# AlexGr5/StereoVision

Hardware: AMD Instinct MI355X
Metric: disparity frames/sec + HBM GB/s, 1920x1080 D=128 win=9, 1/2/4/8 GPU (higher is better)
Workload: dtype u8

## Files before the change

stereovision_amd/csrc/sv_capi_dev.cpp:

```cpp
#include "sv_ctx.h"

extern "C" {

int sv_gray_dev(sv_ctx* c, const uint8_t* d_bgr, int H, int W, int pitch, uint8_t* d_gray, void* stream) {
    SV_ENTER(c);
    if (check_image(d_bgr, H, W) || !d_gray) return fail(SV_EINVAL, "bad gray arguments");
    hipStream_t s = pick(c, stream);
    SV_LAUNCH(c, SV_K_GRAY, s, sv::launch_gray(d_bgr, H, W, pitch, d_gray, s));
    return 0;
}

int sv_disparity_dev(sv_ctx* c, const uint8_t* d_left, const uint8_t* d_right, int H, int W, int pitch,
                     int min_disp, int num_disp, int win, int cost, int row0, int row1, int16_t* d_disp16,
                     int out_pitch, void* stream) {
    SV_ENTER(c);
    if (check_image(d_left, H, W) || check_image(d_right, H, W) || !d_disp16)
        return fail(SV_EINVAL, "bad disparity arguments");
    if (pitch < W || out_pitch < W) return fail(SV_EINVAL, "pitch smaller than width");
    hipStream_t s = pick(c, stream);
    SV_SCRATCH(c, s);
    return enqueue_disparity(c, d_left, d_right, H, W, pitch, min_disp, num_disp, win, cost, row0, row1,
                             d_disp16, out_pitch, s);
}

int sv_median_rows_dev(sv_ctx* c, const int16_t* d_disp16, int H, int W, int row0, int row1, int min_disp,
                       int num_disp, int cost, const sv_map_out* out, void* stream) {
    SV_ENTER(c);
    if (check_image(d_disp16, H, W)) return fail(SV_EINVAL, "bad median arguments");
    if ((long long)H * W >= (1LL << 30)) return fail(SV_EINVAL, "frame too large for the median kernel");
    if (row0 < 0) row0 = 0;
    if (row1 > H) row1 = H;
    hipStream_t s = pick(c, stream);
    SV_SCRATCH(c, s);
    sv::PostParams pp;
    float* disp = nullptr;
    int rc = map_out_post(c, out, min_disp, num_disp, cost, false, s, &pp, &disp);
    if (rc) return rc;
    SV_LAUNCH(c, SV_K_MEDIAN, s, sv::launch_median_i16(d_disp16, H, W, row0, row1, disp, pp, s));
    return 0;
}

int sv_post_m16_dev(sv_ctx* c, const int16_t* d_med16, int64_t n, int mode, float min_depth, float max_depth,
                    float depth_range, float min_disp_global, int min_disp, int num_disp, float* d_disparity,
                    float* d_out_a, uint8_t* d_out_u8, float* d_out_b, void* stream) {
    SV_ENTER(c);
    if (n < 0 || (n > 0 && !d_med16)) return fail(SV_EINVAL, "bad median map");
    if (mode != SV_POST_NONE && mode != SV_POST_DEPTH && mode != SV_POST_SCALED) return fail(SV_EINVAL, "bad mode");
    if (mode == SV_POST_NONE && !d_disparity) return fail(SV_EINVAL, "no outputs");
    if (mode == SV_POST_DEPTH && (!d_out_a || !d_out_u8)) return fail(SV_EINVAL, "depth post outputs missing");
    if (mode == SV_POST_SCALED && (!d_out_a || !d_out_u8 || !d_out_b || num_disp <= 0))
        return fail(SV_EINVAL, "scaled post outputs missing");
    if (n == 0) return 0;
    hipStream_t s = pick(c, stream);
    SV_SCRATCH(c, s);
    sv::PostParams pp = make_post(mode, min_depth, max_depth, depth_range, min_disp_global, min_disp, num_disp,
                                  d_out_a, d_out_u8, d_out_b);
    int rc = attach_lut(c, pp, s);
    if (rc) return rc;
    SV_LAUNCH(c, SV_K_POST, s, sv::launch_post_m16(d_med16, (long long)n, d_disparity, pp, s));
    return 0;
}

int sv_disparity_batch_dev(sv_ctx* c, const uint8_t* d_left, const uint8_t* d_right, int n_frames, int H,
                           int W, int pitch, int64_t frame_stride, int min_disp, int num_disp, int win,
                           int cost, int16_t* d_disp16, int out_pitch, int64_t out_frame_stride,
                           void* stream) {
    SV_ENTER(c);
    if (check_image(d_left, H, W) || check_image(d_right, H, W) || !d_disp16 || n_frames < 0)
        return fail(SV_EINVAL, "bad disparity arguments");
    if (pitch < W || out_pitch < W) return fail(SV_EINVAL, "pitch smaller than width");
    if (n_frames > 1 && (frame_stride < (int64_t)pitch * H || out_frame_stride < (int64_t)out_pitch * H))
        return fail(SV_EINVAL, "frame stride smaller than a frame");
    if (n_frames == 0) return 0;
    hipStream_t s = pick(c, stream);
    SV_SCRATCH(c, s);
    return enqueue_disparity(c, d_left, d_right, H, W, pitch, min_disp, num_disp, win, cost, 0, H, d_disp16,
                             out_pitch, s, n_frames, frame_stride, out_frame_stride);
}

int sv_depth_map_batch_dev(sv_ctx* c, const uint8_t* d_left, const uint8_t* d_right, int n_frames, int H, int W,
                           int pitch, int64_t frame_stride, int min_disp, int num_disp, int win, int cost, int stages,
                           int16_t* d_disp16, const sv_map_out* out, void* stream) {
    SV_ENTER(c);
    if (stages != SV_STAGE_ALL && stages != SV_STAGE_MATCH && stages != SV_STAGE_MEDIAN)
        return fail(SV_EINVAL, "stages must be SV_STAGE_MATCH, SV_STAGE_MEDIAN or SV_STAGE_ALL");
    const bool match = stages & SV_STAGE_MATCH, median = stages & SV_STAGE_MEDIAN;
    if (n_frames < 0 || H <= 0 || W <= 0) return fail(SV_EINVAL, "bad depth-map arguments");
    if (match && (check_image(d_left, H, W) || check_image(d_right, H, W)))
        return fail(SV_EINVAL, "bad depth-map arguments");
    if (!d_disp16 && stages != SV_STAGE_ALL)
        return fail(SV_EINVAL, "the stages run apart exchange the int16 maps through d_disp16");
    if (median && !out) return fail(SV_EINVAL, "null outputs");
    if (median && out->harris && check_image(d_left, H, W)) return fail(SV_EINVAL, "Harris needs the left frames");
    if (pitch < W) return fail(SV_EINVAL, "pitch smaller than width");
    if (n_frames > 1 && frame_stride < (int64_t)pitch * H) return fail(SV_EINVAL, "frame stride smaller than a frame");
    if ((long long)H * W >= (1LL << 30)) return fail(SV_EINVAL, "frame too large for the median kernel");
    if (n_frames == 0) return 0;
    hipStream_t s = pick(c, stream);
    SV_SCRATCH(c, s);
    const long long fs = (long long)H * W;
    int16_t* d16 = d_disp16;
    if (!d16) {
        SV_HIP(c->d16.ensure((size_t)n_frames * fs * sizeof(int16_t)));
        d16 = c->d16.as<int16_t>();
    }
    if (match) {
        const int rc = enqueue_disparity(c, d_left, d_right, H, W, pitch, min_disp, num_disp, win, cost, 0, H, d16, W,
                                         s, n_frames, frame_stride, fs, !d_disp16);
        if (rc) return rc;
    }
    if (!median) return 0;
    sv::PostParams pp;
    float* disp = nullptr;
    int rc = map_out_post(c, out, min_disp, num_disp, cost, true, s, &pp, &disp);
    if (rc) return rc;
    pp.lut_unchecked = match && cost != SV_COST_SGBM && pp.lut_shift == 4 && pp.lut_m0 == (min_disp - 1) * 16 &&
                       pp.lut_n == num_disp + 1;
    const long long fin = n_frames > 1 ? frame_stride : 0;
    if (out->harris && (W < 8 || H < 8)) {
        SV_LAUNCH(c, SV_K_MEDIAN, s, sv::launch_median_i16(d16, H, W, 0, H, disp, pp, s, n_frames, fs, fs));
        SV_LAUNCH(c, SV_K_HARRIS, s, sv::launch_harris(d_left, H, W, pitch, out->harris, s, n_frames, fin, fs));
        return 0;
    }
    sv::HarrisParams hp{d_left, pitch, fin, out->harris, fs, 0, 0};
    SV_LAUNCH(c, SV_K_MEDIAN, s,
              sv::launch_median_i16(d16, H, W, 0, H, disp, pp, s, n_frames, fs, fs, out->harris ? &hp : nullptr));
    return 0;
}

int sv_harris_dev(sv_ctx* c, const uint8_t* d_gray, int H, int W, int pitch, float* d_out, void* stream) {
    SV_ENTER(c);
    if (check_image(d_gray, H, W) || !d_out) return fail(SV_EINVAL, "bad harris arguments");
    hipStream_t s = pick(c, stream);
    SV_LAUNCH(c, SV_K_HARRIS, s, sv::launch_harris(d_gray, H, W, pitch, d_out, s));
    return 0;
}

int sv_harris_batch_dev(sv_ctx* c, const uint8_t* d_gray, int n_frames, int H, int W, int pitch,
                        int64_t frame_stride, float* d_out, void* stream) {
    SV_ENTER(c);
    if (check_image(d_gray, H, W) || !d_out || n_frames < 0) return fail(SV_EINVAL, "bad harris arguments");
    if (pitch < W) return fail(SV_EINVAL, "pitch smaller than width");
    if (n_frames > 1 && frame_stride < (int64_t)pitch * H) return fail(SV_EINVAL, "frame stride smaller than a frame");
    if (n_frames == 0) return 0;
    hipStream_t s = pick(c, stream);
    SV_LAUNCH(c, SV_K_HARRIS, s,
              sv::launch_harris(d_gray, H, W, pitch, d_out, s, n_frames, (long long)frame_stride,
                                (long long)H * W));
    return 0;
}

int sv_hog_hist_dev(sv_ctx* c, const uint8_t* d_gray, int H, int W, int pitch, int win, int row0, int row1,
                    uint16_t* d_out, void* stream) {
    SV_ENTER(c);
    if (check_image(d_gray, H, W) || !d_out) return fail(SV_EINVAL, "bad hog arguments");
    if (win < 1 || win > 15 || (win & 1) == 0) return fail(SV_EINVAL, "win must be odd in [1, 15]");
    hipStream_t s = pick(c, stream);
    SV_LAUNCH(c, SV_K_HOG, s, sv::launch_hog_hist(d_gray, H, W, pitch, win, row0, row1, d_out, s));
    return 0;
}

int sv_gray(sv_ctx* c, const uint8_t* bgr, int H, int W, int stride, uint8_t* gray) {
    SV_ENTER(c);
    SV_SCRATCH(c, c->stream);
    if (check_image(bgr, H, W) || !gray) return fail(SV_EINVAL, "bad gray arguments");
    const size_t row = (size_t)W * 3, n = row * H;
    if (stride < (int)row) return fail(SV_EINVAL, "stride smaller than a row");
    SV_HIP(c->hin.ensure(n));
    for (int y = 0; y < H; ++y) std::memcpy(c->hin.as<uint8_t>() + y * row, bgr + (size_t)y * stride, row);
    SV_HIP(c->img[0].ensure(n));
    SV_HIP(c->gray[0].ensure((size_t)H * W));
    SV_HIP(hipMemcpyAsync(c->img[0].p, c->hin.p, n, hipMemcpyHostToDevice, c->stream));
    SV_LAUNCH(c, SV_K_GRAY, c->stream,
              sv::launch_gray(c->img[0].as<uint8_t>(), H, W, (int)row, c->gray[0].as<uint8_t>(), c->stream));
    Out o[] = {{gray, c->gray[0].p, (size_t)H * W}};
    return collect(c, o, 1);
}

int sv_disparity(sv_ctx* c, const uint8_t* left, const uint8_t* right, int H, int W, int channels, int stride,
                 int min_disp, int num_disp, int win, int cost, int16_t* disp16, float* harris) {
    SV_ENTER(c);
    SV_SCRATCH(c, c->stream);
    if (!disp16) return fail(SV_EINVAL, "null disparity output");
    sv::MatchPlan plan;
    int rc = check_match(H, W, min_disp, num_disp, win, cost, &plan);
    if (rc) return rc;
    rc = stage_pair(c, left, right, H, W, channels, stride);
    if (rc) return rc;
    SV_HIP(c->d16.ensure((size_t)H * W * sizeof(int16_t)));
    rc = enqueue_disparity(c, c->gray[0].as<uint8_t>(), c->gray[1].as<uint8_t>(), H, W, W, min_disp, num_disp,
                           win, cost, 0, H, c->d16.as<int16_t>(), W, c->stream);
    if (rc) return rc;
    if (harris) {
        SV_HIP(c->harris.ensure((size_t)H * W * sizeof(float)));
        SV_LAUNCH(c, SV_K_HARRIS, c->stream,
                  sv::launch_harris(c->gray[0].as<uint8_t>(), H, W, W, c->harris.as<float>(), c->stream));
    }
    Out o[] = {{disp16, c->d16.p, (size_t)H * W * sizeof(int16_t)},
               {harris, c->harris.p, (size_t)H * W * sizeof(float)}};
    return collect(c, o, 2);
}

int sv_disparity_rows(sv_ctx* c, const uint8_t* left, const uint8_t* right, int H, int W, int channels,
                      int stride, int min_disp, int num_disp, int win, int cost, int row0, int row1,
                      int16_t* disp16) {
    SV_ENTER(c);
    SV_SCRATCH(c, c->stream);
    if (!disp16) return fail(SV_EINVAL, "null disparity output");
    if (row0 < 0) row0 = 0;
    if (row1 > H) row1 = H;
    if (row1 <= row0) return 0;
    sv::MatchPlan plan;
    int rc = check_match(H, W, min_disp, num_disp, win, cost, &plan);
    if (rc) return rc;
    rc = stage_pair(c, left, right, H, W, channels, stride);
    if (rc) return rc;
    SV_HIP(c->d16.ensure((size_t)H * W * sizeof(int16_t)));
    rc = enqueue_disparity(c, c->gray[0].as<uint8_t>(), c->gray[1].as<uint8_t>(), H, W, W, min_disp, num_disp,
                           win, cost, row0, row1, c->d16.as<int16_t>(), W, c->stream);
    if (rc) return rc;
    const size_t off = (size_t)row0 * W;
    Out o[] = {{disp16 + off, c->d16.as<int16_t>() + off, (size_t)(row1 - row0) * W * sizeof(int16_t)}};
    return collect(c, o, 1);
}


int sv_median5_f32(sv_ctx* c, const float* in, int H, int W, float* out) {
    SV_ENTER(c);
    SV_SCRATCH(c, c->stream);
    if (check_image(in, H, W) || !out) return fail(SV_EINVAL, "bad median arguments");
    const size_t n = (size_t)H * W * sizeof(float);
    SV_HIP(c->hin.ensure(n));
    SV_HIP(c->fin.ensure(n));
    SV_HIP(c->fa.ensure(n));
    std::memcpy(c->hin.p, in, n);
    SV_HIP(hipMemcpyAsync(c->fin.p, c->hin.p, n, hipMemcpyHostToDevice, c->stream));
    SV_LAUNCH(c, SV_K_MEDIAN, c->stream, sv::launch_median_f32(c->fin.as<float>(), H, W, c->fa.as<float>(), c->stream));
    Out o[] = {{out, c->fa.p, n}};
    return collect(c, o, 1);
}

static int post_common(sv_ctx* c, const float* disparity, int n, const sv::PostParams& tmpl, float* a,
                       uint8_t* u8, float* b) {
    if (!disparity || n <= 0) return fail(SV_EINVAL, "bad post arguments");
    const size_t nb = (size_t)n * sizeof(float);
    SV_HIP(c->hin.ensure(nb));
    SV_HIP(c->fin.ensure(nb));
    SV_HIP(c->fa.ensure(nb));
    SV_HIP(c->fb.ensure(nb));
    SV_HIP(c->u8.ensure((size_t)n));
    std::memcpy(c->hin.p, disparity, nb);
    SV_HIP(hipMemcpyAsync(c->fin.p, c->hin.p, nb, hipMemcpyHostToDevice, c->stream));
    sv::PostParams pp = tmpl;
    pp.out_a = c->fa.as<float>();
    pp.out_u8 = c->u8.as<uint8_t>();
    pp.out_b = c->fb.as<float>();
    SV_LAUNCH(c, SV_K_POST, c->stream, sv::launch_post(c->fin.as<float>(), n, pp, c->stream));
    Out o[] = {{a, c->fa.p, nb}, {u8, c->u8.p, (size_t)n}, {b, c->fb.p, nb}};
    return collect(c, o, 3);
}

int sv_depth_post(sv_ctx* c, const float* disparity, int n, float min_depth, float max_depth, float depth_range,
                  float min_disp_global, float* depth_final, uint8_t* depth_normalized) {
    SV_ENTER(c);
    SV_SCRATCH(c, c->stream);
    if (!depth_final || !depth_normalized) return fail(SV_EINVAL, "null outputs");
    sv::PostParams pp = make_post(SV_POST_DEPTH, min_depth, max_depth, depth_range, min_disp_global, 0, 0,
                                  nullptr, nullptr, nullptr);
    return post_common(c, disparity, n, pp, depth_final, depth_normalized, nullptr);
}

int sv_scaled_post(sv_ctx* c, const float* disparity, int n, int min_disp, int num_disp,
                   float* disparity_normalized, uint8_t* normalized_u8, float* confidence) {
    SV_ENTER(c);
    SV_SCRATCH(c, c->stream);
    if (!disparity_normalized || !normalized_u8 || !confidence || num_disp <= 0)
        return fail(SV_EINVAL, "bad scaled post arguments");
    sv::PostParams pp = make_post(SV_POST_SCALED, 0.f, 0.f, 0.f, 0.f, min_disp, num_disp, nullptr, nullptr,
                                  nullptr);
    return post_common(c, disparity, n, pp, disparity_normalized, normalized_u8, confidence);
}

}

namespace {

std::mutex g_reg_mu;
std::map<uintptr_t, size_t> g_reg;

bool host_registered(const void* p, size_t bytes) {
    if (!p) return false;
    const uintptr_t a = reinterpret_cast<uintptr_t>(p);
    std::lock_guard<std::mutex> lk(g_reg_mu);
    auto it = g_reg.upper_bound(a);
    if (it == g_reg.begin()) return false;
    --it;
    return a >= it->first && a + bytes <= it->first + it->second;
}

int stage_rows(sv_ctx* c, const uint8_t* src, int y0, int y1, size_t row, int stride, uint8_t* stage, uint8_t* dev,
               int nsub) {
    if ((size_t)stride == row) {
        SV_HIP(hipMemcpyAsync(dev + (size_t)y0 * row, src + (size_t)y0 * row, (size_t)(y1 - y0) * row,
                              hipMemcpyHostToDevice, c->stream));
        return 0;
    }
    sv::HostPool& pool = sv::HostPool::get();
    for (int k = 0; k < nsub; ++k) {
        const int a0 = y0 + (int)((long long)(y1 - y0) * k / nsub), a1 = y0 + (int)((long long)(y1 - y0) * (k + 1) / nsub);
        if (a1 <= a0) continue;
        const int parts = pool.threads();
        pool.parallel_for(parts, [&](int p) {
            const int a = a0 + (int)((long long)(a1 - a0) * p / parts), b = a0 + (int)((long long)(a1 - a0) * (p + 1) / parts);
            if (b <= a) return;
            if ((size_t)stride == row)
                std::memcpy(stage + (size_t)a * row, src + (size_t)a * row, (size_t)(b - a) * row);
            else
                for (int y = a; y < b; ++y) std::memcpy(stage + (size_t)y * row, src + (size_t)y * stride, row);
        });
        SV_HIP(hipMemcpyAsync(dev + (size_t)a0 * row, stage + (size_t)a0 * row, (size_t)(a1 - a0) * row,
                              hipMemcpyHostToDevice, c->stream));
    }
    return 0;
}

int host_lut(sv_ctx* c, const sv::PostParams& pp) {
    if (c->hl_valid && c->hl_key == c->lut_key) return 0;
    const size_t n = (size_t)pp.lut_n;
    try {
        c->hl_a.resize(n);
        c->hl_b.resize(n);
        c->hl_u8.resize(n);
    } catch (...) {
        return fail(SV_ENOMEM, "host table allocation failed");
    }
    SV_HIP(hipMemcpyAsync(c->hl_a.data(), pp.lut_a, n * sizeof(float), hipMemcpyDeviceToHost, c->stream));
    SV_HIP(hipMemcpyAsync(c->hl_b.data(), pp.lut_b, n * sizeof(float), hipMemcpyDeviceToHost, c->stream));
    SV_HIP(hipMemcpyAsync(c->hl_u8.data(), pp.lut_u8, n, hipMemcpyDeviceToHost, c->stream));
    SV_HIP(hipStreamSynchronize(c->stream));
    c->hl_key = c->lut_key;
    c->hl_valid = true;
    return 0;
}

struct FrameOut {
    float* a;
    float* disp;
    uint8_t* u8;
    float* b;
    uint8_t* bgr;
};

template <bool U8, bool SCALED, bool BGR>
int expand_rows(const int16_t* med, size_t a, size_t b, int m0, int nl, const HostEnt* ent, const float* lb,
                const FrameOut& o) {
    for (size_t i = a; i < b; ++i) o.disp[i] = (float)med[i] * 0.0625f;
    int nbad = 0;
    for (size_t i = a; i < b; ++i) {
        const uint32_t li = (uint32_t)(med[i] - m0);
        if (__builtin_expect(li >= (uint32_t)nl, 0)) {
            ++nbad;
            continue;
        }
        const HostEnt e = ent[li];
        o.a[i] = e.a;
        if (U8) o.u8[i] = (uint8_t)e.ubgr;
        if (SCALED) o.b[i] = lb[li];
        if (BGR) {
            const uint32_t v = e.ubgr >> 8;
            uint8_t* d = o.bgr + 3 * i;
            if (i + 1 < b) std::memcpy(d, &v, 4);
            else std::memcpy(d, &v, 3);
        }
    }
    return nbad;
}

struct HostProf {
    std::atomic<bool> on{std::getenv("SV_HOST_PROFILE") != nullptr};
    bool print = std::getenv("SV_HOST_PROFILE") != nullptr;
    std::mutex mu;
    double t[6] = {0, 0, 0, 0, 0, 0};
    double acc[6] = {0, 0, 0, 0, 0, 0};
    long n = 0, nacc = 0;
    void add(const double* d) {
        std::lock_guard<std::mutex> lk(mu);
        for (int i = 0; i < 6; ++i) {
            t[i] += d[i];
            acc[i] += d[i];
        }
        ++nacc;
        if (print && ++n % 200 == 0) {
            std::fprintf(stderr, "[sv host] per call (ms): prepare %.3f  stage+issue %.3f  wait-first %.3f  expand %.3f  "
                         "wait-rest %.3f  total %.3f\n", t[0] / n, t[1] / n, t[2] / n, t[3] / n, t[4] / n, t[5] / n);
            for (double& v : t) v = 0;
            n = 0;
        }
    }
};
HostProf& host_prof() {
    static HostProf* p = new HostProf();
    return *p;
}
int env_int(const char* name, int dflt, int lo, int hi) {
    const char* e = std::getenv(name);
    if (!e) return dflt;
    const int v = std::atoi(e);
    return v < lo ? lo : v > hi ? hi : v;
}
double now_ms() {
    return std::chrono::duration<double, std::milli>(std::chrono::steady_clock::now().time_since_epoch()).count();
}

int host_frame_path(sv_ctx* c, const uint8_t* left, const uint8_t* right, int H, int W, int channels, int stride,
                    int min_disp, int num_disp, int win, int cost, sv::PostParams pp, const uint8_t* table,
                    FrameOut o) {
    const bool prof = host_prof().on;
    double tm[6] = {0, 0, 0, 0, 0, 0}, t0 = prof ? now_ms() : 0, tp = t0;
    sv::MatchPlan plan;
    int rc = check_match(H, W, min_disp, num_disp, win, cost, &plan);
// ... 861 lines not shown
```

stereovision_amd/csrc/sv_internal.h:

```cpp
#pragma once
#include <hip/hip_runtime.h>
#include <stdint.h>

#include <cstdlib>
#include <string>

struct sv_comm;

namespace sv {

__device__ __forceinline__ void sad_u32_acc(uint32_t& a, uint32_t b, uint32_t c) {
    asm("v_sad_u32 %0, %0, %1, %2" : "+v"(a) : "v"(b), "v"(c));
}

__device__ __forceinline__ int clampi(int v, int lo, int hi) { return min(max(v, lo), hi); }

__device__ __forceinline__ int bgr_to_gray(int b, int g, int r) {
    return (b * 1868 + g * 9617 + r * 4899 + (1 << 13)) >> 14;
}

inline bool env_flag(const char* name, bool default_on) {
    const char* e = std::getenv(name);
    return default_on ? !(e && e[0] == '0') : (e && e[0] == '1');
}
inline int env_int(const char* name, int lo, int hi) {
    const char* e = std::getenv(name);
    const int v = e ? std::atoi(e) : 0;
    return v >= lo && v <= hi ? v : 0;
}

int set_error(int code, const std::string& msg);

int comm_group_start();
int comm_group_end();
int comm_send(sv_comm* c, const void* buf, size_t bytes, int peer, hipStream_t s);
int comm_recv(sv_comm* c, void* buf, size_t bytes, int peer, hipStream_t s);
int comm_rank(const sv_comm* c);
int comm_size(const sv_comm* c);
int comm_device(const sv_comm* c);

enum Cost { COST_SAD = 0, COST_SSD = 1, COST_HOG = 2, COST_SGBM = 3 };

struct MatchPlan {
    int dpl;
    int lpg;
    int ndw;
    int dbits;
    int mfma_only = 0;
};

struct MatchParams {
    const uint8_t* L;
    const uint8_t* R;
    const uint16_t* HL;
    const uint16_t* HR;
    int H, W, pitch;
    int minD, D, r;
    int win;
    int X0, X1;
    int row0, row1;
    int lpg, lpg_log2, dbits;
    int16_t* out;
    int opitch;
    int nf;
    long long fs_in, fs_out, fs_hist;
    uint32_t pad_key;
    int segm;
    alignas(16) int xcd_map;
    uint32_t* keys;
    long long keys_stride;
    int margins_done;
};

int plan_match(int num_disp, int win, int cost, MatchPlan* plan);
uint64_t max_cost(int win, int cost);
size_t match_lds_bytes(const MatchPlan& p, int r, int cost);
int launch_match(const MatchParams& a, const MatchPlan& p, int cost, hipStream_t s);
bool ring_split(int cost, int win, int num_disp);
bool ring_ssd(int cost, int win, int num_disp);
bool ssd_mfma(int cost, int win, int num_disp);
bool ssd_mfma_fits(const MatchParams& a, int cost);
int launch_ssd_mfma(const MatchParams& a, hipStream_t s);
long long ring_split_elems(int nf, long long fs_out, int row1, int opitch);
int launch_fill_i16(int16_t* out, int opitch, int H, int W, int16_t v, hipStream_t s);

int launch_gray(const uint8_t* bgr, int H, int W, int pitch, uint8_t* gray, hipStream_t s);
int launch_harris(const uint8_t* g, int H, int W, int pitch, float* out, hipStream_t s, int nf = 1,
                  long long fs_in = 0, long long fs_out = 0);
int launch_hog_hist(const uint8_t* g, int H, int W, int pitch, int win, int row0, int row1,
                    uint16_t* hist, hipStream_t s);
int launch_hog_hist_pairs(const uint8_t* g0, const uint8_t* g1, int H, int W, int pitch, int win, int row0,
                          int row1, uint16_t* h0, uint16_t* h1, int nf, long long fs_in, long long fs_hist,
                          hipStream_t s);

struct UndistortParams {
    double ir[9];
    double fx, fy, u0, v0;
    double k[12];
    int H, W;
};
int launch_undistort_map(const UndistortParams& p, short2* map1, uint16_t* map2, hipStream_t s);
int launch_remap(const uint8_t* src, int sH, int sW, int channels, int spitch, long long sfs,
                 const short2* map1, const uint16_t* map2, int H, int W, bool gray_out, uint8_t* dst,
                 int dpitch, long long dfs, int nf, hipStream_t s);

int launch_resize_linear(const void* src, int sH, int sW, int cn, int spitch, long long sfs, void* dst,
                         int dH, int dW, int dpitch, long long dfs, int nf, bool f32, hipStream_t s);

struct FrameStatsArgs {
    const uint8_t* img0;
    const uint8_t* img1;
    int H, W, pitch, cn;
    int bh, bw;
    uint32_t* block_sum;
    uint32_t* block_sq;
    uint32_t* hist;
    uint32_t* hist_copies;
    int per;
    long long fs;
};
constexpr int kHistCopies = 8;
int launch_frame_stats(const FrameStatsArgs& a, int nimg, hipStream_t s);

enum SelectMask { SEL_ALL = 0, SEL_POSITIVE = 1, SEL_MASK_GT = 2 };
constexpr int kMaxRanks = 4;
constexpr int kSelBatch = 16;
struct SelectArgs {
    const float* x;
    const float* mask;
    float thr;
    int mask_mode;
    size_t n;
    int shift, bits;
    int nranks;
    int narr;
    size_t xstride, mstride;
    uint32_t prefix[kSelBatch][kMaxRanks];
    uint32_t* ghist;
    unsigned long long* counts;
    uint32_t* hist_out;
    unsigned long long* counts_out;
};
constexpr int kCountSlots = 32;
int launch_select_hist(const SelectArgs& a, hipStream_t s);

enum AffineMode { AFF_F32 = 0, AFF_F64 = 1, AFF_FILL = 2 };
struct AffineArgs {
    const float* x;
    float* out;
    size_t n;
    int mode;
    float fa, fb, fc, fd;
    double ds, doff;
};
int launch_affine_f32(const AffineArgs& a, hipStream_t s);

struct GaussArgs {
    const float* src;
    float* dst;
    int H, W, r;
    float c[16];
};
enum FuseBase { FUSE_BASE_STEREO = 0, FUSE_BASE_MIDAS = 1, FUSE_BASE_FLOW = 2 };
struct FuseBlendArgs {
    const float* stereo;
    const float* conf;
    const float* midas;
    const float* flow;
    float* fused;
    uint32_t* stats;
    int H, W, base;
    int midas_fill, flow_fill;
    int r;
    float sw, mfw, thr, hthr, k1, k2;
    float c[16];
};
constexpr int kBilateralMaxR = 7;
constexpr int kBilateralMaxTaps = 148;
constexpr int kBilateralLut = 4096 + 2;
struct BilateralArgs {
    const float* src;
    const float* lut;
    float* dst_f32;
    uint8_t* dst_u8;
    uint8_t* dst_bgr;
    const uint32_t* cmap;
    uint32_t* stats;
    int H, W, r, ntaps;
    float scale;
    float sw[kBilateralMaxTaps];
    short off[kBilateralMaxTaps];
};
int bilateral_taps(int r, int* dy, int* dx);
int launch_gauss_f32(const GaussArgs& a, hipStream_t s);
int launch_fuse_blend(const FuseBlendArgs& a, hipStream_t s);
int launch_bilateral_f32(BilateralArgs a, const float* space_w, hipStream_t s);
constexpr int kFuseSlots = 32, kFuseSlotStride = 32;
constexpr size_t kFuseStatsBytes = (size_t)kFuseSlots * kFuseSlotStride * sizeof(uint32_t);
inline void fuse_stats_fold(const uint32_t* slots, uint32_t w[4]) {
    w[0] = w[1] = w[2] = w[3] = 0;
    for (int s = 0; s < kFuseSlots; ++s) {
        const uint32_t* p = slots + s * kFuseSlotStride;
        w[0] = p[0] > w[0] ? p[0] : w[0];
        w[1] = p[1] > w[1] ? p[1] : w[1];
        w[2] += p[2];
        w[3] += p[3];
    }
}
inline float fuse_stat_decode(uint32_t k) {
    const uint32_t u = (k & 0x80000000u) ? (k ^ 0x80000000u) : ~k;
    float f;
    __builtin_memcpy(&f, &u, sizeof f);
    return f;
}
inline float fuse_stat_min(const uint32_t* w) { return fuse_stat_decode(~w[0]); }
inline float fuse_stat_max(const uint32_t* w) { return fuse_stat_decode(w[1]); }

struct SgbmArgs {
    const uint8_t* L;
    const uint8_t* R;
    int H, W, pitch;
    int minD, D, r;
    int Dp;
    int X0, Wb;
    int cap, P1, P2, uniq, disp12;
    uint16_t* hsum;
    uint16_t* C;
    void* Llr;
    void* Lrl;
    void* Ltb;
    int l32;
    int fused;
    uint4* recs;
    void* band;
    int16_t* out;
    int opitch;
    void* dummy;
    long long fs_in, fs_out;
    __device__ __forceinline__ void select_frame(int z) {
        const size_t vol = (size_t)H * Wb * Dp * z;
        L += z * fs_in;
        R += z * fs_in;
        out += z * fs_out;
        hsum += vol;
        C += vol;
        const size_t lb = vol * (l32 ? 4 : 2);
        Llr = static_cast<char*>(Llr) + lb;
        Lrl = static_cast<char*>(Lrl) + lb;
        Ltb = static_cast<char*>(Ltb) + lb;
        band = static_cast<char*>(band) + (size_t)H * Wb * 8 * z;
        if (recs) recs += (size_t)2 * H * W * z;
    }
};
int sgbm_dp(int D);
bool sgbm_fused(int nf, int D);
bool sgbm_cost_fused(int D, int r);
int launch_sgbm(const SgbmArgs& a, int nf, hipStream_t s, hipStream_t aux, hipEvent_t fork, hipEvent_t join);
int launch_speckles(int16_t* img, int H, int W, int pitch, int newv, int maxsize, int maxdiff, int* parent,
                    int* size, hipStream_t s, int nf = 1, long long fimg = 0);

enum PostMode { POST_NONE = 0, POST_DEPTH = 1, POST_SCALED = 2 };
struct PostParams {
    int mode;
    float minf, maxf, rangef, min_disp_global;
    int min_disp, num_disp;
    float* out_a;
    uint8_t* out_u8;
    float* out_b;
    uint8_t* out_bgr;
    const uint32_t* cmap;
    int16_t* out_m16;
    uint8_t* out_d8;
    int d8_base;
    const float* lut_a;
    const uint8_t* lut_u8;
    const float* lut_b;
    int lut_m0, lut_n;
    int lut_shift;
    int lut_unchecked;
    int lut_cap;
};
constexpr int kLutWholeSpan = 4096;
struct HarrisParams {
    const uint8_t* g;
    int pitch;
    long long fs_in;
    float* out;
    long long fs_out;
    int mbx;
    int form;
};
int launch_median_i16(const int16_t* in, int H, int W, int row0, int row1, float* disp,
                      const PostParams& pp, hipStream_t s, int nf = 1, long long fs_in = 0,
                      long long fs_out = 0, const HarrisParams* harris = nullptr);
int launch_median_f32(const float* in, int H, int W, float* out, hipStream_t s);
int launch_post_m16(const int16_t* in, long long n, float* disp, const PostParams& pp, hipStream_t s);
int launch_post(const float* disp, int n, const PostParams& pp, hipStream_t s);
int launch_post_lut(const PostParams& pp, int m0, int n, int step, float* lut_a, uint8_t* lut_u8,
                    float* lut_b, hipStream_t s);

}
```

stereovision_amd/csrc/sv_median.hip:

```cpp
#include <type_traits>
#include "sv_harris_wave.h"
#include "sv_median_net.h"

namespace sv {
namespace {

struct PostVals { float a, b; uint8_t u; };

__device__ __forceinline__ PostVals post_vals(const PostParams& pp, float d) {
    PostVals o{0.0f, 0.0f, 0};
    if (pp.mode == POST_DEPTH) {
        const float fxb = (float)(700 * 0.08);
        const float den = d + (float)1e-6;
        const float depth = fxb / den;
        float dc = depth < pp.minf ? pp.minf : depth;
        dc = dc > pp.maxf ? pp.maxf : dc;
        const bool valid = (d > pp.min_disp_global) && (dc >= pp.minf) && (dc <= pp.maxf);
        o.a = valid ? dc : 0.0f;
        float t = dc - pp.minf;
        t = t / pp.rangef;
        t = t * 255.0f;
        o.u = (uint8_t)(int)t;
    } else if (pp.mode == POST_SCALED) {
        const float lo = (float)pp.min_disp, hi = (float)(pp.min_disp + pp.num_disp - 1);
        float c = d < lo ? lo : d;
        c = c > hi ? hi : c;
        float t = c - lo;
        t = t / (float)pp.num_disp;
        t = t * 255.0f;
        o.u = (uint8_t)(int)t;
        o.a = (float)o.u;
        o.b = (d > (float)(pp.min_disp + 1) && d < hi) ? 1.0f : 0.0f;
    }
    return o;
}

template <typename T>
__device__ __forceinline__ T& at(T* base, uint32_t i) {
    using B = typename std::conditional<std::is_const<T>::value, const char, char>::type;
    return *reinterpret_cast<T*>(reinterpret_cast<B*>(base) + (uint32_t)(i * (uint32_t)sizeof(T)));
}
template <typename T>
__device__ __forceinline__ T& at(T* base, size_t i) { return base[i]; }

template <typename I>
__device__ __forceinline__ void store_post(const PostParams& pp, I i, const PostVals& o) {
    at(pp.out_a, i) = o.a;
    at(pp.out_u8, i) = o.u;
    if (pp.mode == POST_SCALED) at(pp.out_b, i) = o.b;
}

__device__ __forceinline__ void post_one(const PostParams& pp, size_t i, float d) {
    if (pp.mode == POST_NONE) return;
    store_post(pp, i, post_vals(pp, d));
}

typedef short s2 __attribute__((ext_vector_type(2)));
constexpr int MT_W = 64, MT_H = 8;
constexpr int MQ_W = 128, MQ_H = 16;

__device__ __forceinline__ s2 as_s2(uint32_t u) { return __builtin_bit_cast(s2, u); }

__device__ __forceinline__ s2 net_min(s2 a, s2 b) { return __builtin_elementwise_min(a, b); }
__device__ __forceinline__ s2 net_max(s2 a, s2 b) { return __builtin_elementwise_max(a, b); }
__device__ __forceinline__ float net_min(float a, float b) { return fminf(a, b); }
__device__ __forceinline__ float net_max(float a, float b) { return fmaxf(a, b); }
template <typename T, int N, int M>
__device__ __forceinline__ void apply_net(T* v, const unsigned char (&net)[N][M]) {
#pragma unroll
    for (int c = 0; c < N; ++c) {
        const int a = net[c][0], b = net[c][1], use = M == 3 ? net[c][M - 1] : 3;
        const T lo = net_min(v[a], v[b]), hi = net_max(v[a], v[b]);
        if (use & 1) v[a] = lo;
        if (use & 2) v[b] = hi;
    }
}

__device__ __forceinline__ PostVals lut_entry(const PostParams& pp, uint32_t li) {
    PostVals o;
    o.a = at(pp.lut_a, li);
    o.u = at(pp.lut_u8, li);
    o.b = pp.mode == POST_SCALED ? at(pp.lut_b, li) : 0.0f;
    return o;
}
__device__ __forceinline__ PostVals post_median(const PostParams& pp, int mv) {
    const uint32_t dm = (uint32_t)(mv - pp.lut_m0);
    const uint32_t li = dm >> pp.lut_shift;
    if (li < (uint32_t)pp.lut_n && (dm & ((1u << pp.lut_shift) - 1u)) == 0) return lut_entry(pp, li);
    return post_vals(pp, (float)mv / 16.0f);
}
__device__ __forceinline__ PostVals post_median_whole(const PostParams& pp, int mv) {
    return lut_entry(pp, ((uint32_t)(mv - pp.lut_m0) >> 4) & (uint32_t)(kLutWholeSpan - 1));
}

__global__ __launch_bounds__(256) void k_post_m16(const int16_t* __restrict__ in, long long n,
                                                  float* __restrict__ disp, PostParams pp) {
    const long long i0 = ((long long)blockIdx.x * 256 + threadIdx.x) * 8;
    if (i0 >= n) return;
    const bool vec = i0 + 8 <= n && ((((uintptr_t)in) & 15) | (((uintptr_t)disp | (uintptr_t)pp.out_a |
                                                                  (uintptr_t)pp.out_b) & 15) |
                                     ((uintptr_t)pp.out_u8 & 7)) == 0;
    if (vec) {
        const uint4 raw = *reinterpret_cast<const uint4*>(in + i0);
        const uint32_t w[4] = {raw.x, raw.y, raw.z, raw.w};
        int mv[8];
#pragma unroll
        for (int q = 0; q < 4; ++q) {
            mv[2 * q] = (int)(int16_t)(w[q] & 0xFFFFu);
            mv[2 * q + 1] = (int)(int16_t)(w[q] >> 16);
        }
        if (disp) {
            float4* d = reinterpret_cast<float4*>(disp + i0);
            d[0] = make_float4((float)mv[0] / 16.0f, (float)mv[1] / 16.0f, (float)mv[2] / 16.0f, (float)mv[3] / 16.0f);
            d[1] = make_float4((float)mv[4] / 16.0f, (float)mv[5] / 16.0f, (float)mv[6] / 16.0f, (float)mv[7] / 16.0f);
        }
        if (pp.mode == POST_NONE) return;
        PostVals o[8];
#pragma unroll
        for (int q = 0; q < 8; ++q) o[q] = post_median(pp, mv[q]);
        float4* a = reinterpret_cast<float4*>(pp.out_a + i0);
        a[0] = make_float4(o[0].a, o[1].a, o[2].a, o[3].a);
        a[1] = make_float4(o[4].a, o[5].a, o[6].a, o[7].a);
        uint32_t u[2] = {0u, 0u};
#pragma unroll
        for (int q = 0; q < 8; ++q) u[q >> 2] |= (uint32_t)o[q].u << (8 * (q & 3));
        *reinterpret_cast<uint2*>(pp.out_u8 + i0) = make_uint2(u[0], u[1]);
        if (pp.mode == POST_SCALED) {
            float4* b = reinterpret_cast<float4*>(pp.out_b + i0);
            b[0] = make_float4(o[0].b, o[1].b, o[2].b, o[3].b);
            b[1] = make_float4(o[4].b, o[5].b, o[6].b, o[7].b);
        }
        return;
    }
    for (long long i = i0; i < i0 + 8 && i < n; ++i) {
        const int mv = (int)in[i];
        if (disp) disp[i] = (float)mv / 16.0f;
        if (pp.mode == POST_NONE) continue;
        store_post(pp, (size_t)i, post_median(pp, mv));
    }
}

template <int HF, bool WH>
__global__ __launch_bounds__(256) void k_median_i16(const int16_t* __restrict__ in, int H, int W,
                                                    int row0, int row1, float* __restrict__ disp,
                                                    PostParams pp, long long fs_in, long long fs_out,
                                                    HarrisParams hp) {
    if (HF != 0 && (int)blockIdx.x >= hp.mbx) {
        const int w = (int)(blockIdx.x - hp.mbx) * 4 + (int)(threadIdx.x >> 6);
        const int y0 = row0 + (int)blockIdx.y * MQ_H;
        if constexpr (HF == 2) {
            const int x0 = w * 248;
            if (x0 < W && y0 < row1)
                harris_wave4<MQ_H, 4>(hp.g + blockIdx.z * hp.fs_in, H, W, hp.pitch, hp.out + blockIdx.z * hp.fs_out,
                                      x0, y0, threadIdx.x & 63);
        } else {
            const int x0 = w * 60;
            if (x0 < W && y0 < row1)
                harris_wave<MQ_H, 4>(hp.g + blockIdx.z * hp.fs_in, H, W, hp.pitch, hp.out + blockIdx.z * hp.fs_out,
                                     x0, y0, threadIdx.x & 63);
        }
        return;
    }
    constexpr int TC = MQ_W + 4, TR = MQ_H + 2;
    __shared__ uint32_t t2[TR][TC];
    __shared__ __attribute__((aligned(8))) uint32_t srt[MQ_H / 4][4][TC];
    if (blockIdx.z) {
        in += blockIdx.z * fs_in;
        const long long o = blockIdx.z * fs_out;
        if (disp) disp += o;
        if (pp.out_a) pp.out_a += o;
        if (pp.out_u8) pp.out_u8 += o;
        if (pp.out_b) pp.out_b += o;
        if (pp.out_bgr) pp.out_bgr += 3 * o;
        if (pp.out_m16) pp.out_m16 += o;
        if (pp.out_d8) pp.out_d8 += o;
    }
    const int x0 = blockIdx.x * MQ_W, y0 = row0 + blockIdx.y * MQ_H;
    {
        const int c = (int)(threadIdx.x & (MQ_W - 1)), g = (int)(threadIdx.x / MQ_W);
        constexpr int G = 256 / MQ_W;
        static_assert(TR % G == 0, "row groups must tile the pair rows");
        const uint32_t cx = (uint32_t)clampi(x0 - 2 + c, 0, W - 1);
        if (y0 >= 2 && y0 + TR - 1 <= H - 1) {
            uint32_t off = (uint32_t)(y0 - 2 + g) * W + cx;
            const uint32_t two = 2u * (uint32_t)W, step = (uint32_t)G * W;
#pragma unroll
            for (int k = 0; k < TR / G; ++k) {
                const uint16_t a = (uint16_t)at(in, off);
                const uint16_t b = (uint16_t)at(in, off + two);
                t2[g + G * k][c] = (uint32_t)a | ((uint32_t)b << 16);
                off += step;
            }
        } else {
#pragma unroll
            for (int k = 0; k < TR / G; ++k) {
                const int r = g + G * k;
                const uint16_t a = (uint16_t)at(in, (uint32_t)clampi(y0 - 2 + r, 0, H - 1) * W + cx);
                const uint16_t b = (uint16_t)at(in, (uint32_t)clampi(y0 + r, 0, H - 1) * W + cx);
                t2[r][c] = (uint32_t)a | ((uint32_t)b << 16);
            }
        }
        if (threadIdx.x < 4 * TR) {
            const int r = (int)(threadIdx.x >> 2), ce = MQ_W + (int)(threadIdx.x & 3);
            const uint32_t cxe = (uint32_t)clampi(x0 - 2 + ce, 0, W - 1);
            const uint16_t a = (uint16_t)at(in, (uint32_t)clampi(y0 - 2 + r, 0, H - 1) * W + cxe);
            const uint16_t b = (uint16_t)at(in, (uint32_t)clampi(y0 + r, 0, H - 1) * W + cxe);
            t2[r][ce] = (uint32_t)a | ((uint32_t)b << 16);
        }
    }
    __syncthreads();
    const int tx = 2 * (int)(threadIdx.x & 63), tb = 4 * (int)(threadIdx.x >> 6);
    {
        auto sort_col = [&](int g4, int c) {
            s2 w[4];
#pragma unroll
            for (int i = 0; i < 4; ++i) w[i] = as_s2(t2[g4 + 1 + i][c]);
            apply_net(w, SV_SORT4_NET);
#pragma unroll
            for (int i = 0; i < 4; ++i) srt[g4 >> 2][i][c] = __builtin_bit_cast(uint32_t, w[i]);
        };
        sort_col(tb, tx);
        sort_col(tb, tx + 1);
        if (threadIdx.x < 16) sort_col(4 * (threadIdx.x >> 2), MQ_W + (threadIdx.x & 3));
    }
    __syncthreads();

    s2 cm[16], own[2][4];
#pragma unroll
    for (int i = 0; i < 4; ++i) {
        const uint2 p0 = *reinterpret_cast<const uint2*>(&srt[tb >> 2][i][tx]);
        const uint2 p1 = *reinterpret_cast<const uint2*>(&srt[tb >> 2][i][tx + 2]);
        const uint2 p2 = *reinterpret_cast<const uint2*>(&srt[tb >> 2][i][tx + 4]);
        own[0][i] = as_s2(p0.x);
        cm[0 * 4 + i] = as_s2(p0.y);
        cm[1 * 4 + i] = as_s2(p1.x);
        cm[2 * 4 + i] = as_s2(p1.y);
        cm[3 * 4 + i] = as_s2(p2.x);
        own[1][i] = as_s2(p2.y);
    }
    apply_net(cm, SV_SEL16H_NET);
    s2 cw[2][6];
#pragma unroll
    for (int w = 0; w < 2; ++w) {
        s2 z[14];
#pragma unroll
        for (int k = 0; k < 10; ++k) z[k] = cm[SV_SEL16H_OUT[k]];
#pragma unroll
        for (int k = 0; k < 4; ++k) z[10 + k] = own[w][k];
        apply_net(z, SV_MRG14_NET);
#pragma unroll
        for (int k = 0; k < 6; ++k) cw[w][k] = z[SV_MRG14_OUT[k]];
    }
    uint32_t mp[4];
#pragma unroll
    for (int h = 0; h < 2; ++h) {
        s2 q[6];
        {
            const uint2 p0 = *reinterpret_cast<const uint2*>(&t2[tb + 5 * h][tx]);
            const uint2 p1 = *reinterpret_cast<const uint2*>(&t2[tb + 5 * h][tx + 2]);
            const uint2 p2 = *reinterpret_cast<const uint2*>(&t2[tb + 5 * h][tx + 4]);
            q[0] = as_s2(p0.x); q[1] = as_s2(p0.y); q[2] = as_s2(p1.x);
            q[3] = as_s2(p1.y); q[4] = as_s2(p2.x); q[5] = as_s2(p2.y);
        }
        s2 sc[4] = {q[1], q[2], q[3], q[4]};
        apply_net(sc, SV_SORT4_NET);
        s2 m[2];
#pragma unroll
        for (int w = 0; w < 2; ++w) {
            s2 u[5] = {sc[0], sc[1], sc[2], sc[3], w ? q[5] : q[0]};
#pragma unroll
            for (int k = 3; k >= 0; --k) {
                const s2 lo = __builtin_elementwise_min(u[k], u[k + 1]);
                u[k + 1] = __builtin_elementwise_max(u[k], u[k + 1]);
                u[k] = lo;
            }
            s2 r = cw[w][5];
#pragma unroll
            for (int i = 0; i < 5; ++i) r = __builtin_elementwise_min(r, __builtin_elementwise_max(cw[w][i], u[4 - i]));
            m[w] = r;
        }
        const uint32_t a0 = __builtin_bit_cast(uint32_t, m[0]), a1 = __builtin_bit_cast(uint32_t, m[1]);
        mp[h] = (a0 & 0xFFFFu) | (a1 << 16);
        mp[h + 2] = (a0 >> 16) | (a1 & 0xFFFF0000u);
    }
    static_assert(sizeof(srt) >= MQ_H * (MQ_W / 2) * sizeof(uint32_t), "med must fit in srt");
    auto med = reinterpret_cast<uint32_t (*)[MQ_W / 2]>(&srt[0][0][0]);
    __syncthreads();
    med[tb][tx >> 1] = mp[0];
    med[tb + 1][tx >> 1] = mp[1];
    med[tb + 2][tx >> 1] = mp[2];
    med[tb + 3][tx >> 1] = mp[3];
    __syncthreads();
    auto post = [&](int mv) { return WH ? post_median_whole(pp, mv) : post_median(pp, mv); };
    const bool vec = (W & 3) == 0 &&
                     (((uintptr_t)disp | (uintptr_t)pp.out_a | (uintptr_t)pp.out_b) & 15) == 0 &&
                     (((uintptr_t)pp.out_u8 | (uintptr_t)pp.out_bgr | (uintptr_t)pp.out_d8) & 3) == 0 &&
                     ((uintptr_t)pp.out_m16 & 7) == 0;
#pragma unroll
    for (int pass = 0; pass < 2; ++pass) {
        const int r = (int)(threadIdx.x >> 5) + 8 * pass, c4 = (int)(threadIdx.x & 31) * 4;
        const int y = y0 + r, x = x0 + c4;
        if (y >= row1 || x >= W) continue;
        const uint2 raw = *reinterpret_cast<const uint2*>(&med[r][c4 >> 1]);
        const int mv[4] = {(int)(int16_t)(raw.x & 0xFFFF), (int)(int16_t)(raw.x >> 16),
                           (int)(int16_t)(raw.y & 0xFFFF), (int)(int16_t)(raw.y >> 16)};
        const uint32_t i = (uint32_t)y * W + x;
        if (vec) {
            if (disp)
                at(reinterpret_cast<float4*>(disp), i >> 2) =
                    make_float4((float)mv[0] / 16.0f, (float)mv[1] / 16.0f, (float)mv[2] / 16.0f, (float)mv[3] / 16.0f);
            if (pp.out_m16) at(reinterpret_cast<uint2*>(pp.out_m16), i >> 2) = raw;
            if (pp.out_d8)
                at(reinterpret_cast<uint32_t*>(pp.out_d8), i >> 2) =
                    (uint32_t)(uint8_t)((mv[0] >> 4) - pp.d8_base) | ((uint32_t)(uint8_t)((mv[1] >> 4) - pp.d8_base) << 8) |
                    ((uint32_t)(uint8_t)((mv[2] >> 4) - pp.d8_base) << 16) |
                    ((uint32_t)(uint8_t)((mv[3] >> 4) - pp.d8_base) << 24);
            if (pp.mode == POST_NONE) continue;
            PostVals o[4];
#pragma unroll
            for (int q = 0; q < 4; ++q) o[q] = post(mv[q]);
            at(reinterpret_cast<float4*>(pp.out_a), i >> 2) = make_float4(o[0].a, o[1].a, o[2].a, o[3].a);
            at(reinterpret_cast<uint32_t*>(pp.out_u8), i >> 2) =
                (uint32_t)o[0].u | ((uint32_t)o[1].u << 8) | ((uint32_t)o[2].u << 16) | ((uint32_t)o[3].u << 24);
            if (pp.mode == POST_SCALED)
                at(reinterpret_cast<float4*>(pp.out_b), i >> 2) = make_float4(o[0].b, o[1].b, o[2].b, o[3].b);
            if (pp.out_bgr) {
                const uint32_t c0 = pp.cmap[o[0].u], c1 = pp.cmap[o[1].u], c2 = pp.cmap[o[2].u],
                               c3 = pp.cmap[o[3].u];
                uint32_t* d = &at(reinterpret_cast<uint32_t*>(pp.out_bgr), 3 * (i >> 2));
                d[0] = c0 | (c1 << 24);
                d[1] = (c1 >> 8) | (c2 << 16);
                d[2] = (c2 >> 16) | (c3 << 8);
            }
            continue;
        }
#pragma unroll
        for (int q = 0; q < 4; ++q) {
            if (x + q >= W) break;
            if (disp) at(disp, i + q) = (float)mv[q] / 16.0f;
            if (pp.out_m16) at(pp.out_m16, i + q) = (int16_t)mv[q];
            if (pp.out_d8) at(pp.out_d8, i + q) = (uint8_t)((mv[q] >> 4) - pp.d8_base);
            if (pp.mode == POST_NONE) continue;
            const PostVals o = post(mv[q]);
            store_post(pp, i + q, o);
            if (pp.out_bgr) {
                const uint32_t c = pp.cmap[o.u];
                uint8_t* d = &at(pp.out_bgr, 3 * (i + q));
                d[0] = (uint8_t)c;
                d[1] = (uint8_t)(c >> 8);
                d[2] = (uint8_t)(c >> 16);
            }
        }
    }
}

__global__ __launch_bounds__(256) void k_median_f32(const float* __restrict__ in, int H, int W,
                                                    float* __restrict__ out) {
    __shared__ float tile[MT_H + 4][MT_W + 4];
    const int x0 = blockIdx.x * MT_W, y0 = blockIdx.y * MT_H;
    for (int i = threadIdx.x; i < (MT_H + 4) * (MT_W + 4); i += 256) {
        const int ty = i / (MT_W + 4), tx = i % (MT_W + 4);
        tile[ty][tx] = in[(size_t)clampi(y0 - 2 + ty, 0, H - 1) * W + clampi(x0 - 2 + tx, 0, W - 1)];
    }
    __syncthreads();
    const int tx = threadIdx.x % MT_W, pr = threadIdx.x / MT_W;
#pragma unroll
    for (int h = 0; h < 2; ++h) {
        float v[25];
#pragma unroll
        for (int j = 0; j < 5; ++j)
#pragma unroll
            for (int i = 0; i < 5; ++i) v[j * 5 + i] = tile[2 * pr + h + j][tx + i];
        apply_net(v, SV_MED25_NET);
        const int x = x0 + tx, y = y0 + 2 * pr + h;
        if (x < W && y < H) out[(size_t)y * W + x] = v[SV_MED25_OUT];
    }
}

__global__ void k_post(const float* __restrict__ disp, int n, PostParams pp) {
    const int i = blockIdx.x * blockDim.x + threadIdx.x;
    if (i < n) post_one(pp, (size_t)i, disp[i]);
}

__global__ void k_post_lut(PostParams pp, int m0, int n, int step) {
    const int i = blockIdx.x * blockDim.x + threadIdx.x;
    if (i < n) post_one(pp, (size_t)i, (float)(m0 + i * step) / 16.0f);
}

}

int launch_median_i16(const int16_t* in, int H, int W, int row0, int row1, float* disp,
                      const PostParams& pp, hipStream_t s, int nf, long long fs_in, long long fs_out,
                      const HarrisParams* harris) {
    if (row1 <= row0 || nf <= 0) return 0;
    if ((long long)H * W >= (1LL << 30)) return (int)hipErrorInvalidValue;
    HarrisParams hp{};
    int hbx = 0;
    if (harris && harris->g) {
        hp = *harris;
        static const bool med4 = env_flag("SV_HARRIS_MED4", true);
        hp.form = (med4 && W >= 256) ? 1 : 0;
        hbx = hp.form ? ((W + 247) / 248 + 3) / 4 : ((W + 59) / 60 + 3) / 4;
    }
    hp.mbx = (W + MQ_W - 1) / MQ_W;
    const bool wh = pp.lut_unchecked && pp.mode != POST_NONE && pp.lut_shift == 4 && pp.lut_n > 0 &&
                    pp.lut_cap >= kLutWholeSpan;
    void (*fn)(const int16_t*, int, int, int, int, float*, PostParams, long long, long long, HarrisParams) =
        wh ? (hbx == 0 ? k_median_i16<0, true> : hp.form ? k_median_i16<2, true> : k_median_i16<1, true>)
           : (hbx == 0 ? k_median_i16<0, false> : hp.form ? k_median_i16<2, false> : k_median_i16<1, false>);
    hipLaunchKernelGGL(fn, dim3(hp.mbx + hbx, (row1 - row0 + MQ_H - 1) / MQ_H, nf),
                       dim3(256), 0, s, in, H, W, row0, row1, disp, pp, fs_in, fs_out, hp);
    return (int)hipGetLastError();
}

int launch_post_m16(const int16_t* in, long long n, float* disp, const PostParams& pp, hipStream_t s) {
    if (n <= 0) return 0;
    const long long blocks = (n + 8 * 256 - 1) / (8 * 256);
    if (blocks > 0x7FFFFFFFLL) return (int)hipErrorInvalidValue;
    hipLaunchKernelGGL(k_post_m16, dim3((unsigned)blocks), dim3(256), 0, s, in, n, disp, pp);
    return (int)hipGetLastError();
}

int launch_median_f32(const float* in, int H, int W, float* out, hipStream_t s) {
    hipLaunchKernelGGL(k_median_f32, dim3((W + MT_W - 1) / MT_W, (H + MT_H - 1) / MT_H), dim3(256),
                       0, s, in, H, W, out);
    return (int)hipGetLastError();
}

int launch_post_lut(const PostParams& pp, int m0, int n, int step, float* lut_a, uint8_t* lut_u8,
                    float* lut_b, hipStream_t s) {
    if (n <= 0 || pp.mode == POST_NONE) return 0;
    PostParams q = pp;
    q.out_a = lut_a;
    q.out_u8 = lut_u8;
    q.out_b = lut_b;
    q.out_bgr = nullptr;
    q.out_m16 = nullptr;
    q.lut_n = 0;
    hipLaunchKernelGGL(k_post_lut, dim3((n + 255) / 256), dim3(256), 0, s, q, m0, n, step);
    return (int)hipGetLastError();
}

int launch_post(const float* disp, int n, const PostParams& pp, hipStream_t s) {
    if (n <= 0 || pp.mode == POST_NONE) return 0;
    hipLaunchKernelGGL(k_post, dim3((n + 255) / 256), dim3(256), 0, s, disp, n, pp);
    return (int)hipGetLastError();
}

}
```

Measured before the change: 32340.

## Skip median on invalid left band and load median tile as paired dwords

```diff
diff --git a/stereovision_amd/csrc/sv_capi_dev.cpp b/stereovision_amd/csrc/sv_capi_dev.cpp
--- a/stereovision_amd/csrc/sv_capi_dev.cpp
+++ b/stereovision_amd/csrc/sv_capi_dev.cpp
@@ -116,6 +116,7 @@
     if (rc) return rc;
     pp.lut_unchecked = match && cost != SV_COST_SGBM && pp.lut_shift == 4 && pp.lut_m0 == (min_disp - 1) * 16 &&
                        pp.lut_n == num_disp + 1;
+    pp.x_const = pp.lut_unchecked && min_disp + num_disp > 0 ? min_disp + num_disp : 0;
     const long long fin = n_frames > 1 ? frame_stride : 0;
     if (out->harris && (W < 8 || H < 8)) {
         SV_LAUNCH(c, SV_K_MEDIAN, s, sv::launch_median_i16(d16, H, W, 0, H, disp, pp, s, n_frames, fs, fs));
diff --git a/stereovision_amd/csrc/sv_internal.h b/stereovision_amd/csrc/sv_internal.h
--- a/stereovision_amd/csrc/sv_internal.h
+++ b/stereovision_amd/csrc/sv_internal.h
@@ -279,6 +279,7 @@
     int lut_shift;
     int lut_unchecked;
     int lut_cap;
+    int x_const;
 };
 constexpr int kLutWholeSpan = 4096;
 struct HarrisParams {
diff --git a/stereovision_amd/csrc/sv_median.hip b/stereovision_amd/csrc/sv_median.hip
--- a/stereovision_amd/csrc/sv_median.hip
+++ b/stereovision_amd/csrc/sv_median.hip
@@ -140,6 +140,68 @@
     }
 }
 
+template <bool WH, typename F>
+__device__ __forceinline__ void store_medians(const PostParams& pp, float* __restrict__ disp, int W, int row1,
+                                              int x0, int y0, bool vec, F&& raw_of) {
+    auto post = [&](int mv) { return WH ? post_median_whole(pp, mv) : post_median(pp, mv); };
+#pragma unroll
+    for (int pass = 0; pass < 2; ++pass) {
+        const int r = (int)(threadIdx.x >> 5) + 8 * pass, c4 = (int)(threadIdx.x & 31) * 4;
+        const int y = y0 + r, x = x0 + c4;
+        if (y >= row1 || x >= W) continue;
+        const uint2 raw = raw_of(r, c4);
+        const int mv[4] = {(int)(int16_t)(raw.x & 0xFFFF), (int)(int16_t)(raw.x >> 16),
+                           (int)(int16_t)(raw.y & 0xFFFF), (int)(int16_t)(raw.y >> 16)};
+        const uint32_t i = (uint32_t)y * W + x;
+        if (vec) {
+            if (disp)
+                at(reinterpret_cast<float4*>(disp), i >> 2) =
+                    make_float4((float)mv[0] / 16.0f, (float)mv[1] / 16.0f, (float)mv[2] / 16.0f, (float)mv[3] / 16.0f);
+            if (pp.out_m16) at(reinterpret_cast<uint2*>(pp.out_m16), i >> 2) = raw;
+            if (pp.out_d8)
+                at(reinterpret_cast<uint32_t*>(pp.out_d8), i >> 2) =
+                    (uint32_t)(uint8_t)((mv[0] >> 4) - pp.d8_base) | ((uint32_t)(uint8_t)((mv[1] >> 4) - pp.d8_base) << 8) |
+                    ((uint32_t)(uint8_t)((mv[2] >> 4) - pp.d8_base) << 16) |
+                    ((uint32_t)(uint8_t)((mv[3] >> 4) - pp.d8_base) << 24);
+            if (pp.mode == POST_NONE) continue;
+            PostVals o[4];
+#pragma unroll
+            for (int q = 0; q < 4; ++q) o[q] = post(mv[q]);
+            at(reinterpret_cast<float4*>(pp.out_a), i >> 2) = make_float4(o[0].a, o[1].a, o[2].a, o[3].a);
+            at(reinterpret_cast<uint32_t*>(pp.out_u8), i >> 2) =
+                (uint32_t)o[0].u | ((uint32_t)o[1].u << 8) | ((uint32_t)o[2].u << 16) | ((uint32_t)o[3].u << 24);
+            if (pp.mode == POST_SCALED)
+                at(reinterpret_cast<float4*>(pp.out_b), i >> 2) = make_float4(o[0].b, o[1].b, o[2].b, o[3].b);
+            if (pp.out_bgr) {
+                const uint32_t c0 = pp.cmap[o[0].u], c1 = pp.cmap[o[1].u], c2 = pp.cmap[o[2].u],
+                               c3 = pp.cmap[o[3].u];
+                uint32_t* d = &at(reinterpret_cast<uint32_t*>(pp.out_bgr), 3 * (i >> 2));
+                d[0] = c0 | (c1 << 24);
+                d[1] = (c1 >> 8) | (c2 << 16);
+                d[2] = (c2 >> 16) | (c3 << 8);
+            }
+            continue;
+        }
+#pragma unroll
+        for (int q = 0; q < 4; ++q) {
+            if (x + q >= W) break;
+            if (disp) at(disp, i + q) = (float)mv[q] / 16.0f;
+            if (pp.out_m16) at(pp.out_m16, i + q) = (int16_t)mv[q];
+            if (pp.out_d8) at(pp.out_d8, i + q) = (uint8_t)((mv[q] >> 4) - pp.d8_base);
+            if (pp.mode == POST_NONE) continue;
+            const PostVals o = post(mv[q]);
+            store_post(pp, i + q, o);
+            if (pp.out_bgr) {
+                const uint32_t c = pp.cmap[o.u];
+                uint8_t* d = &at(pp.out_bgr, 3 * (i + q));
+                d[0] = (uint8_t)c;
+                d[1] = (uint8_t)(c >> 8);
+                d[2] = (uint8_t)(c >> 16);
+            }
+        }
+    }
+}
+
 template <int HF, bool WH>
 __global__ __launch_bounds__(256) void k_median_i16(const int16_t* __restrict__ in, int H, int W,
                                                     int row0, int row1, float* __restrict__ disp,
@@ -162,7 +224,8 @@
         return;
     }
     constexpr int TC = MQ_W + 4, TR = MQ_H + 2;
-    __shared__ uint32_t t2[TR][TC];
+    static_assert(TC % 2 == 0, "t2's rows must keep 8-byte alignment");
+    __shared__ __attribute__((aligned(8))) uint32_t t2[TR][TC];
     __shared__ __attribute__((aligned(8))) uint32_t srt[MQ_H / 4][4][TC];
     if (blockIdx.z) {
         in += blockIdx.z * fs_in;
@@ -176,12 +239,48 @@
         if (pp.out_d8) pp.out_d8 += o;
     }
     const int x0 = blockIdx.x * MQ_W, y0 = row0 + blockIdx.y * MQ_H;
-    {
+    const bool vec = (W & 3) == 0 &&
+                     (((uintptr_t)disp | (uintptr_t)pp.out_a | (uintptr_t)pp.out_b) & 15) == 0 &&
+                     (((uintptr_t)pp.out_u8 | (uintptr_t)pp.out_bgr | (uintptr_t)pp.out_d8) & 3) == 0 &&
+                     ((uintptr_t)pp.out_m16 & 7) == 0;
+    if (WH && x0 + MQ_W <= pp.x_const) {
+        const uint32_t m2 = (uint32_t)(uint16_t)pp.lut_m0 * 0x10001u;
+        store_medians<WH>(pp, disp, W, row1, x0, y0, vec, [&](int, int) { return make_uint2(m2, m2); });
+        return;
+    }
+    const bool rows_in = y0 >= 2 && y0 + TR - 1 <= H - 1;
+    const bool dwords = WH && rows_in && x0 >= 2 && x0 - 2 + TC <= W && (W & 1) == 0 && ((uintptr_t)in & 3) == 0;
+    if (dwords) {
+        static_assert(TR == 18 && MQ_W == 128, "5 + 5 + 4 + 4 pair rows, 36 entries past 64 dwords");
+        const int wv = __builtin_amdgcn_readfirstlane((int)(threadIdx.x >> 6)), ln = (int)(threadIdx.x & 63);
+        const size_t row = (size_t)(W >> 1);
+        const uint32_t* org = reinterpret_cast<const uint32_t*>(in) + ((size_t)(y0 - 2) * row + (size_t)((x0 - 2) >> 1));
+        const int f = (wv & 1) + 10 * (wv >> 1);
+        const uint32_t* p = org + (size_t)f * row;
+        const bool more = wv < 2, extra = wv == 3 && ln < 2 * TR;
+        const int re = ln >> 1, je = MQ_W / 2 + (ln & 1);
+        uint32_t v[6], ea = 0, eb = 0;
+#pragma unroll
+        for (int i = 0; i < 5; ++i) v[i] = at(p + (size_t)(2 * i) * row, (uint32_t)ln);
+        if (more) v[5] = at(p + 10 * row, (uint32_t)ln);
+        if (extra) {
+            const uint32_t off = (uint32_t)re * (uint32_t)row + (uint32_t)je;
+            ea = at(org, off);
+            eb = at(org, off + 2u * (uint32_t)row);
+        }
+        auto pair_words = [](uint32_t lo, uint32_t hi) {
+            return make_uint2(__builtin_amdgcn_perm(hi, lo, 0x05040100u), __builtin_amdgcn_perm(hi, lo, 0x07060302u));
+        };
+#pragma unroll
+        for (int i = 0; i < 4; ++i) *reinterpret_cast<uint2*>(&t2[f + 2 * i][2 * ln]) = pair_words(v[i], v[i + 1]);
+        if (more) *reinterpret_cast<uint2*>(&t2[f + 8][2 * ln]) = pair_words(v[4], v[5]);
+        if (extra) *reinterpret_cast<uint2*>(&t2[re][2 * je]) = pair_words(ea, eb);
+    } else {
         const int c = (int)(threadIdx.x & (MQ_W - 1)), g = (int)(threadIdx.x / MQ_W);
         constexpr int G = 256 / MQ_W;
         static_assert(TR % G == 0, "row groups must tile the pair rows");
         const uint32_t cx = (uint32_t)clampi(x0 - 2 + c, 0, W - 1);
-        if (y0 >= 2 && y0 + TR - 1 <= H - 1) {
+        if (rows_in) {
             uint32_t off = (uint32_t)(y0 - 2 + g) * W + cx;
             const uint32_t two = 2u * (uint32_t)W, step = (uint32_t)G * W;
 #pragma unroll
@@ -291,67 +390,8 @@
     med[tb + 2][tx >> 1] = mp[2];
     med[tb + 3][tx >> 1] = mp[3];
     __syncthreads();
-    auto post = [&](int mv) { return WH ? post_median_whole(pp, mv) : post_median(pp, mv); };
-    const bool vec = (W & 3) == 0 &&
-                     (((uintptr_t)disp | (uintptr_t)pp.out_a | (uintptr_t)pp.out_b) & 15) == 0 &&
-                     (((uintptr_t)pp.out_u8 | (uintptr_t)pp.out_bgr | (uintptr_t)pp.out_d8) & 3) == 0 &&
-                     ((uintptr_t)pp.out_m16 & 7) == 0;
-#pragma unroll
-    for (int pass = 0; pass < 2; ++pass) {
-        const int r = (int)(threadIdx.x >> 5) + 8 * pass, c4 = (int)(threadIdx.x & 31) * 4;
-        const int y = y0 + r, x = x0 + c4;
-        if (y >= row1 || x >= W) continue;
-        const uint2 raw = *reinterpret_cast<const uint2*>(&med[r][c4 >> 1]);
-        const int mv[4] = {(int)(int16_t)(raw.x & 0xFFFF), (int)(int16_t)(raw.x >> 16),
-                           (int)(int16_t)(raw.y & 0xFFFF), (int)(int16_t)(raw.y >> 16)};
-        const uint32_t i = (uint32_t)y * W + x;
-        if (vec) {
-            if (disp)
-                at(reinterpret_cast<float4*>(disp), i >> 2) =
-                    make_float4((float)mv[0] / 16.0f, (float)mv[1] / 16.0f, (float)mv[2] / 16.0f, (float)mv[3] / 16.0f);
-            if (pp.out_m16) at(reinterpret_cast<uint2*>(pp.out_m16), i >> 2) = raw;
-            if (pp.out_d8)
-                at(reinterpret_cast<uint32_t*>(pp.out_d8), i >> 2) =
-                    (uint32_t)(uint8_t)((mv[0] >> 4) - pp.d8_base) | ((uint32_t)(uint8_t)((mv[1] >> 4) - pp.d8_base) << 8) |
-                    ((uint32_t)(uint8_t)((mv[2] >> 4) - pp.d8_base) << 16) |
-                    ((uint32_t)(uint8_t)((mv[3] >> 4) - pp.d8_base) << 24);
-            if (pp.mode == POST_NONE) continue;
-            PostVals o[4];
-#pragma unroll
-            for (int q = 0; q < 4; ++q) o[q] = post(mv[q]);
-            at(reinterpret_cast<float4*>(pp.out_a), i >> 2) = make_float4(o[0].a, o[1].a, o[2].a, o[3].a);
-            at(reinterpret_cast<uint32_t*>(pp.out_u8), i >> 2) =
-                (uint32_t)o[0].u | ((uint32_t)o[1].u << 8) | ((uint32_t)o[2].u << 16) | ((uint32_t)o[3].u << 24);
-            if (pp.mode == POST_SCALED)
-                at(reinterpret_cast<float4*>(pp.out_b), i >> 2) = make_float4(o[0].b, o[1].b, o[2].b, o[3].b);
-            if (pp.out_bgr) {
-                const uint32_t c0 = pp.cmap[o[0].u], c1 = pp.cmap[o[1].u], c2 = pp.cmap[o[2].u],
-                               c3 = pp.cmap[o[3].u];
-                uint32_t* d = &at(reinterpret_cast<uint32_t*>(pp.out_bgr), 3 * (i >> 2));
-                d[0] = c0 | (c1 << 24);
-                d[1] = (c1 >> 8) | (c2 << 16);
-                d[2] = (c2 >> 16) | (c3 << 8);
-            }
-            continue;
-        }
-#pragma unroll
-        for (int q = 0; q < 4; ++q) {
-            if (x + q >= W) break;
-            if (disp) at(disp, i + q) = (float)mv[q] / 16.0f;
-            if (pp.out_m16) at(pp.out_m16, i + q) = (int16_t)mv[q];
-            if (pp.out_d8) at(pp.out_d8, i + q) = (uint8_t)((mv[q] >> 4) - pp.d8_base);
-            if (pp.mode == POST_NONE) continue;
-            const PostVals o = post(mv[q]);
-            store_post(pp, i + q, o);
-            if (pp.out_bgr) {
-                const uint32_t c = pp.cmap[o.u];
-                uint8_t* d = &at(pp.out_bgr, 3 * (i + q));
-                d[0] = (uint8_t)c;
-                d[1] = (uint8_t)(c >> 8);
-                d[2] = (uint8_t)(c >> 16);
-            }
-        }
-    }
+    store_medians<WH>(pp, disp, W, row1, x0, y0, vec,
+                      [&](int r, int c4) { return *reinterpret_cast<const uint2*>(&med[r][c4 >> 1]); });
 }
 
 __global__ __launch_bounds__(256) void k_median_f32(const float* __restrict__ in, int H, int W,
```

Result: no change. 32420 (median of 6 runs) (+0.2%).
